# CLIAI/speaker-diarization-toolkit

Measured on AMD Instinct MI355X. Metric: segment-embeddings/sec, higher is better.
Workload: dtype bf16; 1 GPU; config #2: 1k synthetic 2-s segments/GPU -> fbank -> ECAPA-TDNN C=1024 -> L2 -> cosine argmax vs 100 profiles; segments_per_gpu=1000, embed_dim=192, weights=random-init seed 0 (20.77 M params), parallelism=segments sharded x1, profiles replicated

## Files before the change

### speaker-diarization-toolkit_amd/csrc/common.hpp

```cpp
#pragma once
#include <hip/hip_runtime.h>
#include <stdint.h>
#include <stdio.h>
#include <vector>

#include "../../include/sdk_hip.h"

typedef __bf16 bf16_t;
typedef __bf16 bf16x8 __attribute__((ext_vector_type(8)));
typedef __bf16 bf16x4 __attribute__((ext_vector_type(4)));
typedef __bf16 bf16x2 __attribute__((ext_vector_type(2)));
typedef float f32x4 __attribute__((ext_vector_type(4)));
typedef float f32x16 __attribute__((ext_vector_type(16)));
typedef uint32_t u32x4 __attribute__((ext_vector_type(4)));
typedef uint32_t u32x2 __attribute__((ext_vector_type(2)));

struct sdk_prof_rec {
  int family;
  hipEvent_t a, b;
  double flops, bytes;
};
struct sdk_ctx {
  int device;
  int num_cu;
  hipDeviceProp_t prop;
  bool prof_on = false;
  bool no_chain_fusion = false;
  bool no_chain_two_per_cu = false;
  bool no_chain_packed = false;
  bool no_asp_packed = false;
  bool no_asp_seg = false;
  bool no_h_kblocked = false;
  int precision = 0;
  int aff_fast = 1;
  void* dbg_ptr = nullptr;
  void* gemm_clk_ptr = nullptr;
  void* gemm_stamps_ptr = nullptr;
  int hp_gemm_variant = 0;
  int matvec_variant = 0;
  int aff_boundary_pen = 0;
  int chol_pivot_rtol_ppb = 1000;
  int chol_shift_ppb = 0;
  bool ahc_distances_only = false;
  bool snorm_scores_only = false;
  bool trials_no_hist = false;
  int aff_variant = 0;
  std::vector<const void*> lds_optin;
  std::vector<sdk_prof_rec> prof;
};

int sdk_lds_optin(sdk_ctx* ctx, const void* func, int bytes);

int asp_fused_launch(sdk_ctx* ctx, const uint16_t* ah, int64_t ldah, const uint16_t* w2, const uint16_t* w2p, const float* b2,
                     const uint16_t* h, int64_t ldh, int B, int T, int C, int A, float* pooled, void* stream, bool kblocked = false, bool f16 = false);

int se_gate_residual_impl(sdk_ctx* ctx, const uint16_t* z, int64_t ldz, const uint16_t* x, int64_t ldx, const float* w1t, const float* b1, const float* w2t,
                          const float* b2, uint16_t* out, int64_t ldo, int B, int T, int C, int Cse, const float* mean_in, void* ws, size_t ws_bytes,
                          void* stream, bool f16);
int asp_stats_impl(sdk_ctx* ctx, const uint16_t* h, int64_t ldh, int B, int T, int C, float* out_ctx, void* stream, bool f16);
int asp_pool_impl(sdk_ctx* ctx, const float* logits, int64_t ldl, const uint16_t* h, int64_t ldh, int B, int T, int C, float* pooled, void* stream, bool f16);

int asp_stats_masked_impl(sdk_ctx* ctx, const uint16_t* h, int64_t ldh, int B, int T, int C, int S, const float* w, const int32_t* valid, float* out_ctx,
                          void* stream, bool f16, int32_t* ok_out);
int asp_pool_masked_impl(sdk_ctx* ctx, const float* logits, int64_t ldl, const uint16_t* h, int64_t ldh, int B, int T, int C, int S, int s, const float* w,
                         const int32_t* valid, float* pooled, void* stream, bool f16);

int res2net_chain_launch(sdk_ctx* ctx, const uint16_t* U, int64_t ldu, uint16_t* R, int64_t ldr, const uint16_t* const* W,
                         const uint16_t* const* Wpk, const float* const* bias, const float* const* scale, const float* const* shift,
                         int nconv, int B, int T, int dil, void* stream, bool f16 = false);

int resnet_tstp_impl(sdk_ctx* ctx, const uint16_t* x, int B, int F, int T, int C, float* out, void* stream, bool f16);
int resnet_masked_tstp_impl(sdk_ctx* ctx, const uint16_t* x, int B, int F, int T, int C, int S, const float* w, const int32_t* valid, float* out,
                            void* stream, bool f16);
int resnet_zero_invalid_impl(sdk_ctx* ctx, float* emb, int n, int dim, const int32_t* valid, void* stream);

size_t ahc_workspace_bytes(const int32_t* offsets, int G);
int ahc_launch(sdk_ctx* ctx, const float* E, int ldE, int dim, const int32_t* offsets, int G, double* Z, int32_t* status, void* ws, void* stream);
int link_launch(sdk_ctx* ctx, const float* E, int ldE, int dim, const int32_t* group, const int32_t* offsets, int G, double stop, double* Z, int32_t* merges,
                int32_t* status, void* ws, void* stream);

struct ProfScope {
  sdk_ctx* c; hipStream_t s; size_t slot; bool on;
  ProfScope(sdk_ctx* ctx, void* stream, int family, double flops, double bytes) : c(ctx), s((hipStream_t)stream), slot(0), on(ctx && ctx->prof_on) {
    if (!on) return;
    sdk_prof_rec r{family, nullptr, nullptr, flops, bytes};
    (void)hipEventCreate(&r.a); (void)hipEventCreate(&r.b);
    (void)hipEventRecord(r.a, s);
    slot = c->prof.size();
    c->prof.push_back(r);
  }
  ~ProfScope() { if (on) (void)hipEventRecord(c->prof[slot].b, s); }
};

void sdk_set_error(const char* fmt, ...) __attribute__((format(printf, 1, 2)));

#define SDK_HIP_OK(expr)                                                              \
  do {                                                                                \
    hipError_t _e = (expr);                                                           \
    if (_e != hipSuccess) {                                                           \
      sdk_set_error("%s failed: %s (%s:%d)", #expr, hipGetErrorString(_e), __FILE__, __LINE__); \
      return 1;                                                                       \
    }                                                                                 \
  } while (0)

#define SDK_REQUIRE(cond, ...)            \
  do {                                    \
    if (!(cond)) {                        \
      sdk_set_error(__VA_ARGS__);         \
      return 2;                           \
    }                                     \
  } while (0)

#define SDK_LAUNCH_CHECK()                                                         \
  do {                                                                             \
    hipError_t _e = hipGetLastError();                                             \
    if (_e != hipSuccess) {                                                        \
      sdk_set_error("kernel launch failed: %s (%s:%d)", hipGetErrorString(_e), __FILE__, __LINE__); \
      return 1;                                                                    \
    }                                                                              \
  } while (0)

static inline int ceil_div(int a, int b) { return (a + b - 1) / b; }

__device__ __forceinline__ float bf16_to_f32(bf16_t v) { return (float)v; }
__device__ __forceinline__ bf16_t f32_to_bf16(float v) { return (bf16_t)v; }

__device__ __forceinline__ float bf16_bits_to_f32(uint32_t lo16) { return __uint_as_float(lo16 << 16); }

__device__ __forceinline__ void unpack8(const u32x4& v, float* f) {
#pragma unroll
  for (int i = 0; i < 4; ++i) {
    f[2 * i] = __uint_as_float(v[i] << 16);
    f[2 * i + 1] = __uint_as_float(v[i] & 0xffff0000u);
  }
}
__device__ __forceinline__ uint32_t pack2(float a, float b) {
  bf16x2 t;
  t[0] = (bf16_t)a;
  t[1] = (bf16_t)b;
  return __builtin_bit_cast(uint32_t, t);
}
typedef _Float16 f16x8_t __attribute__((ext_vector_type(8)));
typedef _Float16 f16x2_t __attribute__((ext_vector_type(2)));
__device__ __forceinline__ float sat_f16(float a) {
  const float c = fminf(fmaxf(a, -65504.f), 65504.f);
  return a != a ? a : c;
}
template <bool F16>
__device__ __forceinline__ uint32_t pack2t(float a, float b) {
  if constexpr (F16) {
    f16x2_t t;
    t[0] = (_Float16)sat_f16(a);
    t[1] = (_Float16)sat_f16(b);
    return __builtin_bit_cast(uint32_t, t);
  } else {
    return pack2(a, b);
  }
}
template <bool F16>
__device__ __forceinline__ void unpack8t(const u32x4& v, float* f) {
  if constexpr (F16) {
#pragma unroll
    for (int i = 0; i < 4; ++i) {
      const uint32_t w = v[i];
      const f16x2_t t = __builtin_bit_cast(f16x2_t, w);
      f[2 * i] = (float)t[0];
      f[2 * i + 1] = (float)t[1];
    }
  } else {
    unpack8(v, f);
  }
}

__device__ __forceinline__ u32x4 pack8(const float* f) {
  u32x4 v;
#pragma unroll
  for (int i = 0; i < 4; ++i) v[i] = pack2(f[2 * i], f[2 * i + 1]);
  return v;
}
template <bool F16>
__device__ __forceinline__ u32x4 pack8t(const float* f) {
  u32x4 v;
#pragma unroll
  for (int i = 0; i < 4; ++i) v[i] = pack2t<F16>(f[2 * i], f[2 * i + 1]);
  return v;
// ... 46 lines not shown
```

### speaker-diarization-toolkit_amd/csrc/conv_gemm.hip

```cpp
#include <stdlib.h>

#include <type_traits>

#include "common.hpp"
#ifndef SDK_GEMM_CHAIN2
#define SDK_GEMM_CHAIN2 2
#endif

namespace {

__device__ __forceinline__ float tanh_bf16(float x) { return 1.0f - __fdividef(2.0f, __expf(2.0f * x) + 1.0f); }

constexpr int BM = 128, BN = 128, BK = 64, NT = 256;
constexpr int LDS_AB = (BM + BN) * BK * 2;
constexpr int CT_STRIDE = (BN + 8) * 2;
constexpr int LDS_CT = BM * CT_STRIDE;
constexpr int LDS_BYTES = LDS_CT > LDS_AB ? LDS_CT : LDS_AB;

struct Params {
  const bf16_t* A; int64_t lda;
  const bf16_t* W;
  bf16_t* C; int64_t ldc;
  float* C32; int64_t ldc32;
  const float* bias; const float* scale; const float* shift;
// ... 37 lines not shown
    m = m < p.M ? m : p.M - 1;
    if (p.taps > 1) {
      const int b = m / p.T;
      segbase[i] = b * p.T;
      tloc[i] = m - b * p.T;
    } else {
      segbase[i] = m;
      tloc[i] = 0;
    }
  }
  const int cpt = p.tap_pack >> 3;
  const int cin_w = p.tap_pack ? BK : p.Cin;
  const int Ktot = p.tap_pack ? ((p.taps * p.tap_pack + BK - 1) / BK) * BK : p.taps * p.Cin;
  const bf16_t* wrow[4];
#pragma unroll
  for (int i = 0; i < 4; ++i) wrow[i] = p.W + (int64_t)(n0 + r0 + 32 * i) * Ktot + ch * 8;

  uint32_t lds_w[4];
#pragma unroll
  for (int i = 0; i < 4; ++i) {
    const int row = r0 + 32 * i;
    lds_w[i] = row * 128 + ((ch ^ (row & 7)) << 4);
  }

  const int ksteps_per_tap = cin_w / BK;
  const int nk = p.tap_pack ? Ktot / BK : p.taps * ksteps_per_tap;
  const int half = p.taps >> 1;

  u32x4 ra[4], rb[4], ra2[4];
  auto gload = [&](int s) {
    const int j = s / ksteps_per_tap;
    const int kc = (s - j * ksteps_per_tap) * BK;
    int off = (j - half) * p.dil, acol = kc + ch * 8;
    if (p.tap_pack) {
      const int g = s * 8 + ch;
      int tap = g / cpt;
      acol = (g - tap * cpt) * 8;
      if (tap >= p.taps) { tap = half; acol = 0; }
      off = (tap - half) * p.dil;
    }
#pragma unroll
    for (int i = 0; i < 4; ++i) {
      const int src = p.taps > 1 ? segbase[i] + reflect_idx(tloc[i] + off, p.T) : segbase[i];
      ra[i] = *reinterpret_cast<const u32x4*>(p.ablk ? p.A + (int64_t)(acol >> 6) * p.ablk + (int64_t)src * 64 + (acol & 63) : p.A + (int64_t)src * p.lda + acol);
      rb[i] = *reinterpret_cast<const u32x4*>(wrow[i] + j * cin_w + kc);
      if (p.A2) ra2[i] = *reinterpret_cast<const u32x4*>(p.A2 + (int64_t)src * p.lda2 + acol);
    }
  };

  f32x4 acc[4][4];
#pragma unroll
  for (int mi = 0; mi < 4; ++mi)
#pragma unroll
    for (int ni = 0; ni < 4; ++ni) acc[mi][ni] = f32x4{0.f, 0.f, 0.f, 0.f};

  const int fr = lane & 15, fq = lane >> 4;
  uint32_t a_off[4], b_off[4];
#pragma unroll
  for (int i = 0; i < 4; ++i) {
    a_off[i] = (wm * 64 + i * 16 + fr) * 128;
    b_off[i] = (wn * 64 + i * 16 + fr) * 128;
  }
  const int sw = lane & 7;

  gload(0);
  for (int s = 0; s < nk; ++s) {
#pragma unroll
    for (int i = 0; i < 4; ++i) {
      if (p.A2) {
        float fa[8], fb[8];
        unpack8t<F16>(ra[i], fa);
        unpack8t<F16>(ra2[i], fb);
#pragma unroll
        for (int e = 0; e < 8; ++e) fa[e] += fb[e];
        ra[i] = pack8t<F16>(fa);
      }
      *reinterpret_cast<u32x4*>(sA + lds_w[i]) = ra[i];
      *reinterpret_cast<u32x4*>(sB + lds_w[i]) = rb[i];
    }
    __syncthreads();
    if (s + 1 < nk) gload(s + 1);
#pragma unroll
    for (int ks = 0; ks < 2; ++ks) {
      const uint32_t coff = ((ks * 4 + fq) ^ sw) << 4;
      bf16x8 af[4], bfr[4];
#pragma unroll
      for (int i = 0; i < 4; ++i) {
        af[i] = *reinterpret_cast<const bf16x8*>(sA + a_off[i] + coff);
        bfr[i] = *reinterpret_cast<const bf16x8*>(sB + b_off[i] + coff);
      }
#pragma unroll
      for (int mi = 0; mi < 4; ++mi)
#pragma unroll
        for (int ni = 0; ni < 4; ++ni)
          acc[mi][ni] = mfma_16x16x32<F16>(af[mi], bfr[ni], acc[mi][ni]);
    }
    __syncthreads();
  }

  float cb[4], cs[4], ct[4];
#pragma unroll
  for (int ni = 0; ni < 4; ++ni) {
    const int col = n0 + wn * 64 + ni * 16 + fr;
    cb[ni] = p.bias ? p.bias[col] : 0.f;
    cs[ni] = p.scale ? p.scale[col] : 1.f;
    ct[ni] = p.shift ? p.shift[col] : 0.f;
  }
  const bool relu = p.flags & SDK_GEMM_RELU, tnh = p.flags & SDK_GEMM_TANH;
#pragma unroll
  for (int mi = 0; mi < 4; ++mi) {
#pragma unroll
    for (int r = 0; r < 4; ++r) {
      const int row = wm * 64 + mi * 16 + fq * 4 + r;
      const int m = m0 + row;
      const float* ub = nullptr;
      if (p.ubias) {
        const int mm = m < p.M ? m : p.M - 1;
        ub = p.ubias + (int64_t)(mm / p.T) * p.ldub;
      }
#pragma unroll
      for (int ni = 0; ni < 4; ++ni) {
        const int lc = wn * 64 + ni * 16 + fr;
        float v = acc[mi][ni][r] + cb[ni];
        if (ub) v += ub[n0 + lc];
        if (relu) v = fmaxf(v, 0.f);
        v = v * cs[ni] + ct[ni];
        if (tnh) v = tanh_bf16(v);
        if (p.C32 && m < p.M) p.C32[(int64_t)m * p.ldc32 + n0 + lc] = v;
        *reinterpret_cast<uint16_t*>(smem + row * CT_STRIDE + lc * 2) = (uint16_t)pack2t<F16>(v, 0.f);
      }
    }
  }
  __syncthreads();
  if (p.C || p.S) {
#pragma unroll
    for (int i = 0; i < 8; ++i) {
      const int id = tid + NT * i;
      const int row = id >> 4, cc = id & 15;
      const int m = m0 + row;
      if (m < p.M) {
        const u32x4 v = *reinterpret_cast<const u32x4*>(smem + row * CT_STRIDE + cc * 16);
        if (p.C) *reinterpret_cast<u32x4*>(p.C + (int64_t)m * p.ldc + n0 + cc * 8) = v;
        if (p.S) {
          const u32x4 x = *reinterpret_cast<const u32x4*>(p.X2 + (int64_t)m * p.ldx2 + n0 + cc * 8);
          float fv[8], fx[8];
          unpack8t<F16>(v, fv);
          unpack8t<F16>(x, fx);
#pragma unroll
          for (int e = 0; e < 8; ++e) fv[e] += fx[e];
          *reinterpret_cast<u32x4*>(p.S + (int64_t)m * p.lds + n0 + cc * 8) = pack8t<F16>(fv);
        }
      }
    }
  }
}

}

namespace {

constexpr int BM2 = 256, BN2 = 256, NT2 = 512;
constexpr int STAGE2 = (BM2 + BN2) * BK * 2;
constexpr int LDS2 = 2 * STAGE2;
constexpr int LDS2_PAR = LDS2 + 3 * BN2 * 4;
constexpr int LDS2_TOTAL = LDS2_PAR + 8 * 2 * BN2 * 4;
static_assert(BM2 * BN2 * 2 <= LDS2, "the bf16 image of a finished tile must fit in the two pipeline stages");

typedef const void __attribute__((address_space(1)))* gptr_t;
typedef void __attribute__((address_space(3)))* lptr_t;

template <bool TAPS, bool CKB = false, bool F16 = false>
__global__ __launch_bounds__(NT2, 2) void conv_gemm256_kernel(Params p) {
  extern __shared__ __attribute__((aligned(16))) char smem[];
  const int tid = threadIdx.x, lane = tid & 63, wid = tid >> 6;
  const unsigned long long clk_c0 = p.clk ? __builtin_amdgcn_s_memtime() : 0, clk_r0 = p.clk ? __builtin_amdgcn_s_memrealtime() : 0;
  const int wm = wid >> 2, wn = wid & 3;

  const int nbn = p.N / BN2;
  const int nbm = (p.M + BM2 - 1) / BM2;
  const int ntiles = nbn * nbm;
  const int cpt = p.tap_pack >> 3;
  const int cin_w = p.tap_pack ? BK : p.Cin;
  const int Ktot = p.tap_pack ? ((p.taps * p.tap_pack + BK - 1) / BK) * BK : p.taps * p.Cin;
  const int ksteps_per_tap = cin_w / BK;
  const int nk = p.tap_pack ? Ktot / BK : p.taps * ksteps_per_tap;
  const int half = p.taps >> 1;

  const int G = gridDim.x;
  const bool unit_order = !(p.tune & 64) && G == 256 && (nbn & 3) == 0 && nbm >= 64;
  const int xcd = blockIdx.x & 7, slot = blockIdx.x >> 3;
  const int nch = nbn >> 2, mg_full = nbm >> 3;
  const int full_units = mg_full * nch, R = full_units >> 3, rem_units = full_units - 8 * R;
  const int gm_tail = nbm & 7, tail_tiles = gm_tail * nbn;
  const int mt0 = unit_order && (8 * R) % nch == 0 ? ((8 * R) / nch) * 8 : 0;
  const int n_half_m = 2 * (nbm - mt0);
  const int half_cap = 32 / nbn;
  const bool half_tail = unit_order && !(p.tune & 512) && (8 * R) % nch == 0 && R > 0 && mt0 < nbm && n_half_m <= 8 * half_cap;
  const int nrounds = unit_order ? (half_tail ? R : R + (rem_units + (tail_tiles + 31) / 32 + 7) / 8) : (ntiles + G - 1) / G;
  auto tile_coords = [&](int i, int& tm0, int& tn0) -> bool {
    if (unit_order) {
      int u;
      if (i < R) {
        u = xcd * R + i;
      } else {
        const int q = (i - R) * 8 + xcd;
        if (q >= rem_units) {
          const int pj = (q - rem_units) * 32 + slot;
          if (pj >= tail_tiles) return false;
          tm0 = (mg_full * 8 + pj % gm_tail) * BM2;
          tn0 = (pj / gm_tail) * BN2;
          return true;
        }
        u = 8 * R + q;
      }
      const int mg = u / nch, ch = u - mg * nch;
      tm0 = (mg * 8 + (slot & 7)) * BM2;
      tn0 = (ch * 4 + (slot >> 3)) * BN2;
      return true;
    }
    const int vt = blockIdx.x + G * i;
    if (vt >= ntiles) return false;
    const int tile = xcd_remap(vt, ntiles);
    constexpr int GM = 8;
    const int per_group = GM * nbn;
    const int grp = tile / per_group, in_grp = tile - grp * per_group;
    const int gm = min(nbm - grp * GM, GM);
    tm0 = (grp * GM + in_grp % gm) * BM2;
    tn0 = (in_grp / gm) * BN2;
    return true;
  };

  const int rin = lane >> 3, pos = lane & 7;
  const int gch = (pos ^ rin) * 8;
  const int wu = __builtin_amdgcn_readfirstlane(wid);
  const bool a_nt = !TAPS && nbn <= 4;
  uint32_t aoff[4];
  int aseg0 = 0, atl0 = 0;
  uint32_t woff;
  auto setup_dma = [&](int tm0, int tn0, auto ap_c) {
    constexpr int AP = decltype(ap_c)::value;
    const int row = 8 * AP * wu + rin;
    if constexpr (TAPS) {
      const int mm = min(tm0 + row, p.M - 1);
      aseg0 = (mm / p.T) * p.T;
      atl0 = mm - aseg0;
    } else {
#pragma unroll
      for (int i = 0; i < AP; ++i) aoff[i] = ((uint32_t)min(tm0 + row + 8 * i, p.M - 1) * (uint32_t)p.lda + (uint32_t)gch) * 2u;
    }
    woff = ((uint32_t)(tn0 + 32 * wu + rin) * (uint32_t)Ktot + (uint32_t)gch) * 2u;
  };
  auto issue = [&](int t, int stage, auto ap_c) {
    constexpr int AP = decltype(ap_c)::value;
    const int j = t / ksteps_per_tap;
    const int kc = (t - j * ksteps_per_tap) * BK;
    char* sA = smem + stage * STAGE2 + (8 * AP * wu) * 128;
    char* sB = smem + stage * STAGE2 + BM2 * BK * 2 + (32 * wu) * 128;
    const char* abase = reinterpret_cast<const char*>(p.A + kc);
    if constexpr (TAPS) {
      int off = (j - half) * p.dil;
      uint32_t acol = (uint32_t)gch;
      if (p.tap_pack) {
        const int g = t * 8 + (gch >> 3);
        int tap = g / cpt;
        acol = (uint32_t)(g - tap * cpt) * 8u;
        if (tap >= p.taps) { tap = half; acol = 0; }
        off = (tap - half) * p.dil;
      }
#pragma unroll
      for (int i = 0; i < AP; ++i) {
        int tl = atl0 + 8 * i, sb = aseg0;
        if (tl >= p.T) { tl -= p.T; sb += p.T; }
        const uint32_t src = (uint32_t)min(sb + reflect_idx(tl + off, p.T), p.M - 1);
        __builtin_amdgcn_global_load_lds((gptr_t)(abase + (size_t)((src * (uint32_t)p.lda + acol) * 2u)), (lptr_t)(sA + i * 1024), 16, 0, 0);
      }
    } else if (a_nt) {
#pragma unroll
      for (int i = 0; i < AP; ++i)
        __builtin_amdgcn_global_load_lds((gptr_t)(abase + (size_t)aoff[i]), (lptr_t)(sA + i * 1024), 16, 0, 2);
    } else {
#pragma unroll
      for (int i = 0; i < AP; ++i)
        __builtin_amdgcn_global_load_lds((gptr_t)(abase + (size_t)aoff[i]), (lptr_t)(sA + i * 1024), 16, 0, 0);
    }
    const char* wbase = reinterpret_cast<const char*>(p.W + (j * cin_w + kc));
#pragma unroll
    for (int i = 0; i < 4; ++i)
      __builtin_amdgcn_global_load_lds((gptr_t)(wbase + (size_t)i * 16 * Ktot + (size_t)woff), (lptr_t)(sB + i * 1024), 16, 0, 0);
  };
  constexpr std::integral_constant<int, 4> kWhole{};
  constexpr std::integral_constant<int, 2> kHalf{};

  const int fr = lane & 15, fq = lane >> 4, sw = lane & 7;
  const uint32_t a_base = (wm * 128 + fr) * 128;
  const uint32_t b_base = BM2 * BK * 2 + (wn * 64 + fr) * 128;
  const uint32_t c0 = ((0 * 4 + fq) ^ sw) << 4, c1 = ((1 * 4 + fq) ^ sw) << 4;
  const bool dma_early = wu < 4;
  const bool relu = p.flags & SDK_GEMM_RELU;
  const bool stats = p.stats_part != nullptr;
  float* par = reinterpret_cast<float*>(smem + LDS2);

  int nst = 0;
  auto stamp = [&]() {
    if (p.stamps && blockIdx.x == 0 && tid == 0 && nst < 4096) p.stamps[nst++] = __builtin_amdgcn_s_memrealtime();
  };
  auto ldB = [&](const char* st, bf16x8* dst, uint32_t coff) {
// ... 418 lines not shown
      bf16_t* dst = CKB ? p.C + (int64_t)((n0 >> 6) + (cc >> 3)) * p.cblk + (int64_t)(m0 + r0) * 64 + (cc & 7) * 8
                        : p.C + (int64_t)(m0 + r0) * p.ldc + n0 + cc * 8;
      const int64_t ldc = CKB ? 64 : p.ldc;
      const int rows_left = p.M - m0 - r0;
#pragma unroll
      for (int i = 0; i < 8; ++i) {
        if (16 * i < rows_left) {
          const u32x4 v = *reinterpret_cast<const u32x4*>(src + i * 16 * (BN2 * 2));
          __builtin_nontemporal_store(v, reinterpret_cast<u32x4*>(dst + (int64_t)(16 * i) * ldc));
        }
      }
    }
    if (stats) tile_stats((m0 / BM2) * BM2, m0 & 128, 128, n0);
    stamp();
    }
  }
  if (p.clk && tid == 0 && blockIdx.x < 4096) {
    p.clk[blockIdx.x * 2] = __builtin_amdgcn_s_memtime() - clk_c0;
    p.clk[blockIdx.x * 2 + 1] = __builtin_amdgcn_s_memrealtime() - clk_r0;
  }
}

__global__ __launch_bounds__(256) void colstats_finish_kernel(const float* __restrict__ part, int M, int N, int T, int mode,
                                                             float* __restrict__ out) {
  const int b = blockIdx.x, n = blockIdx.y * 256 + threadIdx.x;
  if (n >= N) return;
  const int64_t nbm = (M + BM2 - 1) / BM2;
  const int r_lo = b * T, r_hi = (b + 1) * T - 1;
  float s = 0.f, q = 0.f;
  for (int t = r_lo / BM2; t <= r_hi / BM2; ++t) {
    const int slot = b - (t * BM2) / T;
    const float* ps = part + ((int64_t)(t * 2) * 3 + slot) * N + n;
    s += ps[0];
    s += ps[3 * (int64_t)N];
    if (mode == 2) {
      const float* pq = ps + nbm * 6 * N;
      q += pq[0];
      q += pq[3 * (int64_t)N];
    }
  }
  const float invT = 1.0f / (float)T;
  const float mean = s * invT;
  if (mode == 1) {
    out[(int64_t)b * N + n] = mean;
  } else {
    out[(int64_t)b * 2 * N + n] = mean;
    out[(int64_t)b * 2 * N + N + n] = sqrtf(var_floor(q * invT - mean * mean));
  }
}

int g_gemm_variant = -1;

}

extern "C" size_t sdk_conv_gemm_stats_bytes(int M, int N, int mode) {
  if (M <= 0 || N <= 0 || mode < 1 || mode > 2) return 0;
  return (size_t)((M + BM2 - 1) / BM2) * 6 * (size_t)N * sizeof(float) * (size_t)mode;
}

extern "C" int sdk_conv_gemm_stats_fusable(int M, int N, int T) {
  return ((g_gemm_variant < 0 ? 2 : g_gemm_variant) & 15) != 1 && N % BN2 == 0 && M >= BM2 && T >= 128;
}

extern "C" int sdk_colstats_finish(sdk_ctx* ctx, const float* stats_part, int M, int N, int T, int mode, float* out, void* stream) {
  SDK_REQUIRE(ctx && stats_part && out, "sdk_colstats_finish: null argument");
  SDK_REQUIRE(M > 0 && T > 0 && M % T == 0 && (mode == 1 || mode == 2), "sdk_colstats_finish: bad shape");
  hipLaunchKernelGGL(colstats_finish_kernel, dim3(M / T, ceil_div(N, 256)), dim3(256), 0, (hipStream_t)stream, stats_part, M, N, T, mode, out);
  SDK_LAUNCH_CHECK();
  return 0;
}

extern "C" int sdk_set_gemm_variant(int v) {
  g_gemm_variant = v;
  return 0;
}

extern "C" int sdk_conv_gemm(sdk_ctx* ctx, const sdk_conv_gemm_args* a, void* stream) {
  SDK_REQUIRE(ctx && a, "sdk_conv_gemm: null ctx/args");
  SDK_REQUIRE(a->A && a->W, "sdk_conv_gemm: A and W are required");
  SDK_REQUIRE(a->M > 0 && a->N > 0 && a->N % BN == 0, "sdk_conv_gemm: N=%d must be a positive multiple of %d", a->N, BN);
  const int pack = a->tap_pack;
  if (pack) {
    SDK_REQUIRE(pack > 0 && pack % 8 == 0 && a->taps > 1 && !a->A2 && a->Cin == pack, "sdk_conv_gemm: tap_pack=%d needs taps > 1, a multiple of 8 channels per tap, Cin == tap_pack and no A2", pack);
  } else
  SDK_REQUIRE(a->Cin > 0 && a->Cin % BK == 0, "sdk_conv_gemm: Cin=%d must be a multiple of %d", a->Cin, BK);
  SDK_REQUIRE(a->taps >= 1 && (a->taps & 1), "sdk_conv_gemm: taps=%d must be odd", a->taps);
  SDK_REQUIRE(a->T > 0 && a->M % a->T == 0, "sdk_conv_gemm: M=%d must be a multiple of T=%d", a->M, a->T);
  SDK_REQUIRE((int64_t)a->N * a->taps * a->Cin < (1ll << 31), "sdk_conv_gemm: weight matrix of %d x %d elements exceeds 2^31", a->N, a->taps * a->Cin);
  SDK_REQUIRE(a->taps == 1 || (a->taps / 2) * a->dil < a->T, "sdk_conv_gemm: segment of T=%d frames shorter than the conv halo %d", a->T, (a->taps / 2) * a->dil);
  const bool a_kb = (a->flags & SDK_GEMM_A_KBLOCKED) != 0, c_kb = (a->flags & SDK_GEMM_C_KBLOCKED) != 0, f16 = (a->flags & SDK_GEMM_F16) != 0;
  if (a_kb) SDK_REQUIRE(a->taps == 1 && !pack && !a->A2, "sdk_conv_gemm: a K-blocked A operand needs taps == 1, no tap packing and no A2");
  else
  SDK_REQUIRE(a->lda % 8 == 0 && a->lda >= a->Cin, "sdk_conv_gemm: lda=%lld must be >= Cin and a multiple of 8", (long long)a->lda);
  SDK_REQUIRE(((uintptr_t)a->A % 16) == 0 && ((uintptr_t)a->W % 16) == 0, "sdk_conv_gemm: A/W must be 16-byte aligned");
  SDK_REQUIRE(a->C || a->C32 || a->S, "sdk_conv_gemm: no output requested");
  if (a->C && !c_kb) SDK_REQUIRE(a->ldc % 8 == 0 && a->ldc >= a->N && ((uintptr_t)a->C % 16) == 0, "sdk_conv_gemm: bad C/ldc");
  if (c_kb) SDK_REQUIRE(a->C && ((uintptr_t)a->C % 16) == 0, "sdk_conv_gemm: a K-blocked output needs C (16-byte aligned)");
  if (a->S) SDK_REQUIRE(a->X2 && a->lds % 8 == 0 && a->ldx2 % 8 == 0 && ((uintptr_t)a->S % 16) == 0 && ((uintptr_t)a->X2 % 16) == 0, "sdk_conv_gemm: S needs X2 and 16-byte aligned rows");
  if (a->C32) SDK_REQUIRE(a->ldc32 >= a->N, "sdk_conv_gemm: bad ldc32");
  if (a->ubias) SDK_REQUIRE(a->ldub >= a->N, "sdk_conv_gemm: bad ldub");

  if (g_gemm_variant < 0) {
    const char* e = getenv("SDK_GEMM_VARIANT");
    g_gemm_variant = e ? atoi(e) : 2;
  }
  if (sdk_lds_optin(ctx, (const void*)conv_gemm256_kernel<false>, LDS2_TOTAL)) return 1;
  if (sdk_lds_optin(ctx, (const void*)conv_gemm256_kernel<true>, LDS2_TOTAL)) return 1;
  if (sdk_lds_optin(ctx, (const void*)conv_gemm256_kernel<false, true>, LDS2_TOTAL)) return 1;
  if (sdk_lds_optin(ctx, (const void*)conv_gemm256_kernel<false, false, true>, LDS2_TOTAL)) return 1;
  if (sdk_lds_optin(ctx, (const void*)conv_gemm256_kernel<true, false, true>, LDS2_TOTAL)) return 1;
  if (sdk_lds_optin(ctx, (const void*)conv_gemm256_kernel<false, true, true>, LDS2_TOTAL)) return 1;
  Params p;
  p.A = (const bf16_t*)a->A; p.lda = a->lda; p.W = (const bf16_t*)a->W;
  p.C = (bf16_t*)a->C; p.ldc = a->ldc; p.C32 = a->C32; p.ldc32 = a->ldc32;
  p.bias = a->bias; p.scale = a->scale; p.shift = a->shift; p.ubias = a->ubias; p.ldub = a->ldub;
  p.X2 = (const bf16_t*)a->X2; p.ldx2 = a->ldx2; p.S = (bf16_t*)a->S; p.lds = a->lds;
  p.M = a->M; p.N = a->N; p.Cin = a->Cin; p.taps = a->taps; p.dil = a->dil; p.T = a->T; p.flags = a->flags;
  p.tune = g_gemm_variant / 16;
  p.stats_part = nullptr; p.stats_mode = 0;
  p.A2 = (const bf16_t*)a->A2; p.lda2 = a->lda2;
  p.tap_pack = pack;
  p.ablk = a_kb ? (int64_t)a->M * 64 : 0;
  p.cblk = c_kb ? (int64_t)a->M * 64 : 0;
  p.clk = (unsigned long long*)ctx->gemm_clk_ptr;
  p.stamps = (unsigned long long*)ctx->gemm_stamps_ptr;
  if (a->A2) SDK_REQUIRE(a->lda2 % 8 == 0 && a->lda2 >= a->Cin && ((uintptr_t)a->A2 % 16) == 0, "sdk_conv_gemm: bad A2/lda2");

  const double kk = pack ? (double)(((a->taps * pack + BK - 1) / BK) * BK) : (double)a->taps * a->Cin;
  const bool use256 = !a_kb && ((g_gemm_variant & 15) != 1 || c_kb) && a->N % BN2 == 0 && a->M >= BM2 && !a->A2 && a->C && !a->C32 && !a->S &&
                      !a->ubias && !(a->flags & SDK_GEMM_TANH) && (a->taps == 1 || a->T >= 64) &&
                      (uint64_t)a->M * (uint64_t)a->lda * 2u < (1ull << 32);
  ProfScope ps(ctx, stream, use256 ? SDK_K_CONV_GEMM256 : SDK_K_CONV_GEMM, 2.0 * a->M * a->N * kk,
               2.0 * a->M * a->Cin + 2.0 * a->N * kk + (a->C ? 2.0 : 0.0) * a->M * a->N + (a->C32 ? 4.0 : 0.0) * a->M * a->N +
                   (a->S ? 4.0 : 0.0) * a->M * a->N);
  if (c_kb) SDK_REQUIRE(use256 && a->taps == 1, "sdk_conv_gemm: a K-blocked output needs the plain-layer shape of the 256^2 kernel (taps == 1, N %% 256 == 0, M >= 256, bf16 output only)");
  if (a->stats_mode) {
    SDK_REQUIRE(a->stats_mode == 1 || a->stats_mode == 2, "sdk_conv_gemm: stats_mode=%d", a->stats_mode);
    SDK_REQUIRE(use256 && a->T >= 128 && a->stats_part && a->C, "sdk_conv_gemm: fused column statistics need the 256^2 kernel (N %% 256 == 0, M >= 256), T >= 128 and a bf16 output");
    p.stats_part = a->stats_part; p.stats_mode = a->stats_mode;
  }
  if (use256) {
    const int ntiles = (a->N / BN2) * ceil_div(a->M, BM2);
    const int cus = ctx->num_cu > 0 ? (ctx->num_cu / 8) * 8 : 256;
    const int grid = (p.tune & 8) ? ntiles : (ntiles < cus ? ntiles : cus);
    if (f16) {
      void (*kern)(Params) = conv_gemm256_kernel<false, false, true>;
      if (c_kb) kern = conv_gemm256_kernel<false, true, true>;
      else if (p.taps > 1) kern = conv_gemm256_kernel<true, false, true>;
      hipLaunchKernelGGL(kern, dim3(grid), dim3(NT2), LDS2_TOTAL, (hipStream_t)stream, p);
    } else if (c_kb)
      hipLaunchKernelGGL((conv_gemm256_kernel<false, true>), dim3(grid), dim3(NT2), LDS2_TOTAL, (hipStream_t)stream, p);
    else
      hipLaunchKernelGGL(p.taps > 1 ? conv_gemm256_kernel<true> : conv_gemm256_kernel<false>, dim3(grid), dim3(NT2), LDS2_TOTAL, (hipStream_t)stream, p);
  } else {
    hipLaunchKernelGGL(f16 ? conv_gemm_kernel<true> : conv_gemm_kernel<false>, dim3((a->N / BN) * ceil_div(a->M, BM)), dim3(NT), LDS_BYTES, (hipStream_t)stream, p);
  }
  SDK_LAUNCH_CHECK();
  return 0;
}
```

### speaker-diarization-toolkit_amd/csrc/sdk_api.hip

```cpp
#include <stdarg.h>
#include <string.h>

#include "common.hpp"
#include "ecapa_layout.h"
#include "hp.hpp"

static thread_local char g_err[512] = "";

void sdk_set_error(const char* fmt, ...) {
  va_list ap;
  va_start(ap, fmt);
  vsnprintf(g_err, sizeof(g_err), fmt, ap);
  va_end(ap);
}

extern "C" const char* sdk_last_error(void) { return g_err; }
extern "C" int sdk_abi_version(void) { return SDK_ABI_VERSION; }

extern "C" int sdk_init(int device, sdk_ctx** out) {
  SDK_REQUIRE(out, "sdk_init: out is null");
  *out = nullptr;
  int n = 0;
  hipError_t e = hipGetDeviceCount(&n);
  if (e != hipSuccess || n <= 0) {
    sdk_set_error("sdk_init: no HIP device available (%s); this library has no CPU fallback",
                  e != hipSuccess ? hipGetErrorString(e) : "device count is 0");
    return 1;
  }
  SDK_REQUIRE(device >= 0 && device < n, "sdk_init: device %d out of range (0..%d)", device, n - 1);
  sdk_ctx* c = new sdk_ctx();
  c->device = device;
  if (hipGetDeviceProperties(&c->prop, device) != hipSuccess) {
    delete c;
    sdk_set_error("sdk_init: hipGetDeviceProperties failed");
    return 1;
  }
  if (strncmp(c->prop.gcnArchName, "gfx950", 6) != 0) {
    sdk_set_error("sdk_init: device %d is %s; libsdk_hip.so carries gfx950 (MI355X) code objects only", device,
                  c->prop.gcnArchName);
    delete c;
    return 1;
  }
  c->num_cu = c->prop.multiProcessorCount;
  SDK_HIP_OK(hipSetDevice(device));
  *out = c;
  return 0;
}

int sdk_lds_optin(sdk_ctx* ctx, const void* func, int bytes) {
  for (const void* f : ctx->lds_optin)
    if (f == func) return 0;
  SDK_HIP_OK(hipSetDevice(ctx->device));
  SDK_HIP_OK(hipFuncSetAttribute(func, hipFuncAttributeMaxDynamicSharedMemorySize, bytes));
  ctx->lds_optin.push_back(func);
  return 0;
}

extern "C" int sdk_device_malloc(sdk_ctx* ctx, size_t bytes, void** out) {
  SDK_REQUIRE(ctx && out, "sdk_device_malloc: null argument");
  *out = nullptr;
  SDK_HIP_OK(hipSetDevice(ctx->device));
  SDK_HIP_OK(hipMalloc(out, bytes ? bytes : 1));
  return 0;
}
extern "C" int sdk_device_free(sdk_ctx* ctx, void* p) {
  SDK_REQUIRE(ctx, "sdk_device_free: null context");
  if (p) SDK_HIP_OK(hipFree(p));
  return 0;
}
extern "C" int sdk_memcpy(sdk_ctx* ctx, void* dst, const void* src, size_t bytes, int kind, void* stream) {
  SDK_REQUIRE(ctx && (bytes == 0 || (dst && src)), "sdk_memcpy: null argument");
  SDK_REQUIRE(kind >= 1 && kind <= 3, "sdk_memcpy: kind=%d (1 = host to device, 2 = device to host, 3 = device to device)", kind);
  if (!bytes) return 0;
  const hipMemcpyKind k = kind == 1 ? hipMemcpyHostToDevice : kind == 2 ? hipMemcpyDeviceToHost : hipMemcpyDeviceToDevice;
  SDK_HIP_OK(hipMemcpyAsync(dst, src, bytes, k, (hipStream_t)stream));
  SDK_HIP_OK(hipStreamSynchronize((hipStream_t)stream));
  return 0;
}
extern "C" int sdk_stream_synchronize(sdk_ctx* ctx, void* stream) {
  SDK_REQUIRE(ctx, "sdk_stream_synchronize: null context");
  SDK_HIP_OK(hipStreamSynchronize((hipStream_t)stream));
  return 0;
}

extern "C" int sdk_shutdown(sdk_ctx* ctx) {
  delete ctx;
  return 0;
}

extern "C" int sdk_get_device_info(sdk_ctx* ctx, sdk_device_info* out) {
  SDK_REQUIRE(ctx && out, "sdk_get_device_info: null argument");
  memset(out, 0, sizeof(*out));
  out->device = ctx->device;
  out->compute_units = ctx->prop.multiProcessorCount;
  out->clock_khz = ctx->prop.clockRate;
  out->wavefront_size = ctx->prop.warpSize;
  out->hbm_bytes = ctx->prop.totalGlobalMem;
  strncpy(out->name, ctx->prop.name, sizeof(out->name) - 1);
  strncpy(out->arch, ctx->prop.gcnArchName, sizeof(out->arch) - 1);
  return 0;
}

extern "C" int sdk_set_option(sdk_ctx* ctx, const char* name, int value) {
  SDK_REQUIRE(ctx && name, "sdk_set_option: null argument");
  if (strcmp(name, "res2net_chain_fusion") == 0) { ctx->no_chain_fusion = value == 0; return 0; }
  if (strcmp(name, "res2net_packed_weights") == 0) { ctx->no_chain_packed = value == 0; return 0; }
  if (strcmp(name, "res2net_two_per_cu") == 0) { ctx->no_chain_two_per_cu = value == 0; return 0; }
  if (strcmp(name, "asp_packed_weights") == 0) { ctx->no_asp_packed = value == 0; return 0; }
  if (strcmp(name, "asp_per_segment") == 0) { ctx->no_asp_seg = value == 0; return 0; }
  if (strcmp(name, "h_kblocked") == 0) { ctx->no_h_kblocked = value == 0; return 0; }
  if (strcmp(name, "precision") == 0) {
    SDK_REQUIRE(value >= 0 && value <= 2, "sdk_set_option: precision must be 0 (bf16 operands), 1 (fp16 hi+lo planes) or 2 (one fp16 plane), got %d", value);
    ctx->precision = value;
    return 0;
  }
  if (strcmp(name, "gemm_variant") == 0) return sdk_set_gemm_variant(value);
  if (strcmp(name, "affinity_fast_path") == 0) { ctx->aff_fast = value; return 0; }
  if (strcmp(name, "affinity_variant") == 0) { ctx->aff_variant = value; return 0; }
  if (strcmp(name, "affinity_boundary_penalty") == 0) { ctx->aff_boundary_pen = value < 0 ? 0 : value; return 0; }
  if (strcmp(name, "matvec_variant") == 0) { ctx->matvec_variant = value; return 0; }
  if (strcmp(name, "hp_gemm_variant") == 0) { ctx->hp_gemm_variant = value; return 0; }
  if (strcmp(name, "affinity_whole_groups") == 0) return 0;
  if (strcmp(name, "chol_pivot_rtol_ppb") == 0) { ctx->chol_pivot_rtol_ppb = value < 0 ? 0 : value; return 0; }
  if (strcmp(name, "chol_shift_ppb") == 0) { ctx->chol_shift_ppb = value < 0 ? 0 : value; return 0; }
  if (strcmp(name, "ahc_distances_only") == 0) { ctx->ahc_distances_only = value != 0; return 0; }
  if (strcmp(name, "snorm_scores_only") == 0) { ctx->snorm_scores_only = value != 0; return 0; }
  if (strcmp(name, "trials_no_hist") == 0) { ctx->trials_no_hist = value != 0; return 0; }
  sdk_set_error("sdk_set_option: unknown option '%s'", name);
  return 2;
}

extern "C" int sdk_debug_set_ptr(sdk_ctx* ctx, const char* name, void* p) {
  SDK_REQUIRE(ctx && name, "sdk_debug_set_ptr: null argument");
  if (strcmp(name, "stamps") == 0) { ctx->dbg_ptr = p; return 0; }
  if (strcmp(name, "gemm_clock") == 0) { ctx->gemm_clk_ptr = p; return 0; }
  if (strcmp(name, "gemm_stamps") == 0) { ctx->gemm_stamps_ptr = p; return 0; }
  sdk_set_error("sdk_debug_set_ptr: unknown name '%s'", name);
  return 2;
}

extern "C" int sdk_profile_begin(sdk_ctx* ctx) {
  SDK_REQUIRE(ctx, "sdk_profile_begin: null ctx");
  for (auto& r : ctx->prof) { (void)hipEventDestroy(r.a); (void)hipEventDestroy(r.b); }
  ctx->prof.clear();
  ctx->prof_on = true;
  return 0;
}

extern "C" int sdk_profile_end(sdk_ctx* ctx, sdk_profile_report* out) {
  SDK_REQUIRE(ctx && out, "sdk_profile_end: null argument");
  ctx->prof_on = false;
  memset(out, 0, sizeof(*out));
  SDK_HIP_OK(hipDeviceSynchronize());
  for (auto& r : ctx->prof) {
    float ms = 0.f;
    SDK_HIP_OK(hipEventElapsedTime(&ms, r.a, r.b));
    if (r.family >= 0 && r.family < SDK_K_COUNT) {
      out->launches[r.family] += 1;
      out->ms[r.family] += ms;
      out->flops[r.family] += r.flops;
      out->bytes[r.family] += r.bytes;
    }
    (void)hipEventDestroy(r.a);
    (void)hipEventDestroy(r.b);
  }
  ctx->prof.clear();
  return 0;
}

namespace {

inline size_t a256(size_t v) { return (v + 255) & ~(size_t)255; }

struct FwdWs {
  uint16_t *X0, *U, *R, *Z, *Sa, *Sb, *CAT, *H, *AH;
  float *ctx, *ubias, *logits, *pooled, *se, *stats, *mean;
};

size_t fwd_layout(const sdk_ecapa_desc* d, int B, int T, char* base, FwdWs* w, bool full_logits = false) {
  const size_t M = (size_t)B * T, C = d->channels, Cm = d->mfa_channels, S = d->sub_channels, A = d->attn_channels;
  size_t off = 0;
  auto take = [&](size_t bytes) { char* p = base ? base + off : nullptr; off += a256(bytes); return p; };
  char* x0 = take(M * C * 2);
  char* u = take(M * C * 2);
  char* r = take(M * C * 2);
  char* z = take(M * C * 2);
  char* sa = take(M * S * 2);
  char* sb = take(M * S * 2);
  char* cat = take(M * Cm * 2);
  char* h = take(M * Cm * 2);
  char* ah = take(M * A * 2);
  char* cx = take((size_t)B * 2 * Cm * 4);
  char* ub = take((size_t)B * A * 4);
  const bool fused_asp = !full_logits && A == 128 && T <= sdk_asp_fused_max_frames();
  char* lg = take(fused_asp ? 256 : M * Cm * 4);
  char* po = take((size_t)B * 2 * Cm * 4);
  char* se = take(sdk_se_workspace_bytes(B, (int)C, d->se_channels));
  char* stp = take(sdk_conv_gemm_stats_bytes((int)M, (int)Cm, 2));
  char* mn = take((size_t)B * C * 4);
  if (w) { w->se = (float*)se; w->stats = (float*)stp; w->mean = (float*)mn; }
  if (w) {
    w->X0 = (uint16_t*)x0; w->U = (uint16_t*)u; w->R = (uint16_t*)r; w->Z = (uint16_t*)z;
    w->Sa = (uint16_t*)sa; w->Sb = (uint16_t*)sb; w->CAT = (uint16_t*)cat; w->H = (uint16_t*)h; w->AH = (uint16_t*)ah;
    w->ctx = (float*)cx; w->ubias = (float*)ub; w->logits = (float*)lg; w->pooled = (float*)po;
  }
  return off;
}

struct FwdWsHp {
  uint16_t *X0, *U, *R, *Z, *Sa, *Sb, *CAT, *H, *AH;
  float *ctx, *ubias, *logits, *pooled, *mean, *hid, *gate;
};

size_t fwd_layout_hp(const sdk_ecapa_desc* d, int B, int T, char* base, FwdWsHp* w) {
  const size_t M = (size_t)B * T, C = d->channels, Cm = d->mfa_channels, S = d->sub_channels, A = d->attn_channels;
  size_t off = 0;
  auto take = [&](size_t bytes) { char* p = base ? base + off : nullptr; off += a256(bytes); return p; };
  char* x0 = take(M * C * 4);
  char* u = take(M * C * 4);
  char* r = take(M * C * 4);
  char* z = take(M * C * 4);
  char* sa = take(M * S * 4);
  char* sb = take(M * S * 4);
  char* cat = take(M * Cm * 4);
  char* h = take(M * Cm * 4);
  char* ah = take(M * A * 4);
  char* cx = take((size_t)B * 2 * Cm * 4);
  char* ub = take((size_t)B * A * 4);
  char* lg = take(M * Cm * 4);
  char* po = take((size_t)B * 2 * Cm * 4);
  char* mn = take((size_t)B * C * 4);
  char* hd = take((size_t)B * d->se_channels * 4);
  char* gt = take((size_t)B * C * 4);
  if (w) {
    w->X0 = (uint16_t*)x0; w->U = (uint16_t*)u; w->R = (uint16_t*)r; w->Z = (uint16_t*)z; w->Sa = (uint16_t*)sa; w->Sb = (uint16_t*)sb;
    w->CAT = (uint16_t*)cat; w->H = (uint16_t*)h; w->AH = (uint16_t*)ah; w->ctx = (float*)cx; w->ubias = (float*)ub; w->logits = (float*)lg;
    w->pooled = (float*)po; w->mean = (float*)mn; w->hid = (float*)hd; w->gate = (float*)gt;
  }
  return off;
}

int check_desc(const sdk_ecapa_desc* d) {
  SDK_REQUIRE(d, "ecapa desc is null");
  SDK_REQUIRE(d->n_blocks >= 1 && d->n_blocks <= 4, "ecapa desc: n_blocks=%d", d->n_blocks);
  SDK_REQUIRE(d->channels % 128 == 0 && d->mfa_channels == d->n_blocks * d->channels, "ecapa desc: channels=%d mfa=%d", d->channels, d->mfa_channels);
  SDK_REQUIRE(d->scale >= 2 && d->sub_channels * d->scale == d->channels && d->sub_channels % 128 == 0, "ecapa desc: res2net scale=%d sub=%d", d->scale, d->sub_channels);
  SDK_REQUIRE(d->attn_channels % 128 == 0 && d->n_mels_padded % (d->precision == 1 ? 32 : 64) == 0, "ecapa desc: attn=%d mels=%d", d->attn_channels, d->n_mels_padded);
  SDK_REQUIRE((d->kernel0 & 1) == 1, "ecapa desc: kernel0=%d must be odd", d->kernel0);
  SDK_REQUIRE(d->precision >= 0 && d->precision <= 2, "ecapa desc: precision=%d", d->precision);
  return 0;
}

int ecapa_forward_hp(sdk_ctx* ctx, const void* wblob, const sdk_ecapa_desc* d, const uint16_t* feats, int ldf, int B, int T, void* ws,
                     float* emb, void* stream) {
  FwdWsHp w;
  fwd_layout_hp(d, B, T, (char*)ws, &w);
  const char* wb = (const char*)wblob;
  auto P16 = [&](int slot) -> const uint16_t* { return d->off[slot] < 0 ? nullptr : (const uint16_t*)(wb + d->off[slot]); };
  auto P32 = [&](int slot) -> const float* { return d->off[slot] < 0 ? nullptr : (const float*)(wb + d->off[slot]); };
  const int M = B * T, C = d->channels, Cm = d->mfa_channels, S = d->sub_channels, A = d->attn_channels;
  const int flo = ldf >> 1;
  SDK_REQUIRE(ldf % 16 == 0 && flo >= d->n_mels_padded, "sdk_ecapa_forward: precise mode takes feature planes, ldf=%d must be >= 2 x %d", ldf, d->n_mels_padded);

// ... 614 lines not shown
```

Baseline: 121,400 segment-embeddings/sec.

## Add persistent double-buffered skinny GEMM kernel for N=128 convolutions

```diff
diff --git a/speaker-diarization-toolkit_amd/csrc/common.hpp b/speaker-diarization-toolkit_amd/csrc/common.hpp
--- a/speaker-diarization-toolkit_amd/csrc/common.hpp
+++ b/speaker-diarization-toolkit_amd/csrc/common.hpp
@@ -31,6 +31,7 @@
   bool no_asp_packed = false;
   bool no_asp_seg = false;
   bool no_h_kblocked = false;
+  bool no_skinny_gemm = false;
   int precision = 0;
   int aff_fast = 1;
   void* dbg_ptr = nullptr;
diff --git a/speaker-diarization-toolkit_amd/csrc/conv_gemm.hip b/speaker-diarization-toolkit_amd/csrc/conv_gemm.hip
--- a/speaker-diarization-toolkit_amd/csrc/conv_gemm.hip
+++ b/speaker-diarization-toolkit_amd/csrc/conv_gemm.hip
@@ -213,6 +213,183 @@
         }
       }
     }
+  }
+}
+
+constexpr int SK_LDS = 2 * LDS_AB;
+static_assert(BM * BN * 2 <= LDS_AB, "the 2-byte image of a finished tile must fit in one pipeline stage");
+
+template <bool F16>
+__global__ __launch_bounds__(NT, 2) void conv_gemm_skinny_kernel(Params p) {
+  extern __shared__ __attribute__((aligned(16))) char smem[];
+  const int tid = threadIdx.x;
+  const int lane = tid & 63;
+  const int wid = tid >> 6;
+  const int wm = wid >> 1, wn = wid & 1;
+
+  const int ntiles = (p.M + BM - 1) / BM;
+  const int G = gridDim.x;
+  const int nk = p.Cin / BK;
+  const int total = ((ntiles - (int)blockIdx.x + G - 1) / G) * nk;
+
+  const int ch = tid & 7;
+  const int r0 = tid >> 3;
+  const uint32_t lds_w0 = r0 * 128 + ((ch ^ (r0 & 7)) << 4);
+  const int64_t arow = p.ablk ? 64 : p.lda;
+  const int64_t astep_live = p.ablk ? p.ablk : BK;
+
+  const bf16_t* pa[4];
+  int64_t astep = 0;
+  int a_vt = blockIdx.x, a_k = 0;
+  auto a_tile = [&]() __attribute__((always_inline)) {
+    const bool live = a_vt < ntiles;
+    const int m0 = live ? xcd_remap(a_vt, ntiles) * BM : 0;
+    astep = live ? astep_live : 0;
+#pragma unroll
+    for (int i = 0; i < 4; ++i) {
+      int m = m0 + r0 + 32 * i;
+      m = m < p.M ? m : p.M - 1;
+      pa[i] = p.A + (live ? (int64_t)m * arow : 0) + ch * 8;
+    }
+  };
+  auto a_issue = [&](u32x4* dst) __attribute__((always_inline)) {
+#pragma unroll
+    for (int i = 0; i < 4; ++i) {
+      dst[i] = *reinterpret_cast<const u32x4*>(pa[i]);
+      pa[i] += astep;
+    }
+    if (++a_k == nk) { a_k = 0; a_vt += G; a_tile(); }
+  };
+  a_tile();
+  const bf16_t* const w0 = p.W + (int64_t)r0 * p.Cin + ch * 8;
+  const int64_t wrow32 = (int64_t)32 * p.Cin;
+  int w_k = 0;
+  auto w_issue = [&](u32x4* dst) __attribute__((always_inline)) {
+#pragma unroll
+    for (int i = 0; i < 4; ++i) dst[i] = *reinterpret_cast<const u32x4*>(w0 + i * wrow32 + w_k * BK);
+    w_k = w_k + 1 == nk ? 0 : w_k + 1;
+  };
+  auto lds_fill = [&](char* stage, const u32x4* a, const u32x4* b) __attribute__((always_inline)) {
+#pragma unroll
+    for (int i = 0; i < 4; ++i) *reinterpret_cast<u32x4*>(stage + lds_w0 + i * 4096) = a[i];
+    __builtin_amdgcn_sched_barrier(0);
+#pragma unroll
+    for (int i = 0; i < 4; ++i) *reinterpret_cast<u32x4*>(stage + BM * BK * 2 + lds_w0 + i * 4096) = b[i];
+    __builtin_amdgcn_sched_barrier(0);
+  };
+
+  f32x4 acc[4][4];
+#pragma unroll
+  for (int mi = 0; mi < 4; ++mi)
+#pragma unroll
+    for (int ni = 0; ni < 4; ++ni) acc[mi][ni] = f32x4{0.f, 0.f, 0.f, 0.f};
+
+  const int fr = lane & 15, fq = lane >> 4;
+  uint32_t a_off[4], b_off[4];
+#pragma unroll
+  for (int i = 0; i < 4; ++i) {
+    a_off[i] = (wm * 64 + i * 16 + fr) * 128;
+    b_off[i] = BM * BK * 2 + (wn * 64 + i * 16 + fr) * 128;
+  }
+  const int sw = lane & 7;
+
+  const bool relu = p.flags & SDK_GEMM_RELU, tnh = p.flags & SDK_GEMM_TANH;
+
+  auto epilogue = [&](int m0, char* img) __attribute__((always_inline)) {
+    float cb[4], cs[4], ct[4];
+#pragma unroll
+    for (int ni = 0; ni < 4; ++ni) {
+      const int col = wn * 64 + ni * 16 + fr;
+      cb[ni] = p.bias ? p.bias[col] : 0.f;
+      cs[ni] = p.scale ? p.scale[col] : 1.f;
+      ct[ni] = p.shift ? p.shift[col] : 0.f;
+    }
+    const bool has_ub = p.ubias != nullptr;
+#pragma unroll
+    for (int mi = 0; mi < 4; ++mi) {
+      float ubv[4][4];
+#pragma unroll
+      for (int r = 0; r < 4; ++r) {
+        const int m = m0 + wm * 64 + mi * 16 + fq * 4 + r;
+        const int mm = m < p.M ? m : p.M - 1;
+        const float* ub = has_ub ? p.ubias + (int64_t)(mm / p.T) * p.ldub : nullptr;
+#pragma unroll
+        for (int ni = 0; ni < 4; ++ni) ubv[r][ni] = has_ub ? ub[wn * 64 + ni * 16 + fr] : 0.f;
+      }
+#pragma unroll
+      for (int r = 0; r < 4; ++r) {
+        const int row = wm * 64 + mi * 16 + fq * 4 + r;
+#pragma unroll
+        for (int ni = 0; ni < 4; ++ni) {
+          const int lc = wn * 64 + ni * 16 + fr;
+          float v = acc[mi][ni][r] + cb[ni];
+          if (has_ub) v += ubv[r][ni];
+          if (relu) v = fmaxf(v, 0.f);
+          v = v * cs[ni] + ct[ni];
+          if (tnh) v = tanh_bf16(v);
+          *reinterpret_cast<uint16_t*>(img + row * 256 + (((lc >> 3) ^ (fq << 1)) << 4) + (lc & 7) * 2) = (uint16_t)pack2t<F16>(v, 0.f);
+          acc[mi][ni][r] = 0.f;
+        }
+      }
+    }
+    lds_barrier();
+#pragma unroll
+    for (int i = 0; i < 8; ++i) {
+      const int id = tid + NT * i;
+      const int row = id >> 4, cc = id & 15;
+      const int m = m0 + row;
+      if (m < p.M) {
+        const u32x4 v = *reinterpret_cast<const u32x4*>(img + row * 256 + ((cc ^ (((row >> 2) & 3) << 1)) << 4));
+        *reinterpret_cast<u32x4*>(p.C + (int64_t)m * p.ldc + cc * 8) = v;
+      }
+    }
+    lds_barrier();
+  };
+
+  u32x4 ra[2][4], rb[4];
+  int c_vt = blockIdx.x, c_k = 0;
+  auto step = [&](auto par_c) __attribute__((always_inline)) {
+    constexpr int P = decltype(par_c)::value;
+    char* st = smem + P * LDS_AB;
+    lds_fill(smem + (P ^ 1) * LDS_AB, ra[P ^ 1], rb);
+    w_issue(rb);
+    a_issue(ra[P ^ 1]);
+    __builtin_amdgcn_sched_barrier(0);
+#pragma unroll
+    for (int ks = 0; ks < 2; ++ks) {
+      const uint32_t coff = ((ks * 4 + fq) ^ sw) << 4;
+      bf16x8 af[4], bfr[4];
+#pragma unroll
+      for (int i = 0; i < 4; ++i) {
+        af[i] = *reinterpret_cast<const bf16x8*>(st + a_off[i] + coff);
+        bfr[i] = *reinterpret_cast<const bf16x8*>(st + b_off[i] + coff);
+      }
+#pragma unroll
+      for (int mi = 0; mi < 4; ++mi)
+#pragma unroll
+        for (int ni = 0; ni < 4; ++ni)
+          acc[mi][ni] = mfma_16x16x32<F16>(af[mi], bfr[ni], acc[mi][ni]);
+    }
+    lds_barrier();
+    if (++c_k == nk && c_vt < ntiles) {
+      epilogue(xcd_remap(c_vt, ntiles) * BM, st);
+      c_k = 0;
+      c_vt += G;
+    }
+  };
+  constexpr std::integral_constant<int, 0> kEven{};
+  constexpr std::integral_constant<int, 1> kOdd{};
+
+  a_issue(ra[0]);
+  w_issue(rb);
+  a_issue(ra[1]);
+  lds_fill(smem, ra[0], rb);
+  w_issue(rb);
+  a_issue(ra[0]);
+  lds_barrier();
+  for (int g = 0; g < total; g += 2) {
+    step(kEven);
+    step(kOdd);
   }
 }
 
@@ -937,6 +1114,11 @@
       hipLaunchKernelGGL((conv_gemm256_kernel<false, true>), dim3(grid), dim3(NT2), LDS2_TOTAL, (hipStream_t)stream, p);
     else
       hipLaunchKernelGGL(p.taps > 1 ? conv_gemm256_kernel<true> : conv_gemm256_kernel<false>, dim3(grid), dim3(NT2), LDS2_TOTAL, (hipStream_t)stream, p);
+  } else if (!ctx->no_skinny_gemm && a->N == BN && a->taps == 1 && !pack && !a->A2 && !a->X2 && !a->S && !a->C32 && a->C && !a->stats_mode) {
+    const int ntiles = ceil_div(a->M, BM);
+    const int slots = 2 * (ctx->num_cu >= 8 ? (ctx->num_cu / 8) * 8 : 256);
+    hipLaunchKernelGGL(f16 ? conv_gemm_skinny_kernel<true> : conv_gemm_skinny_kernel<false>, dim3(ntiles < slots ? ntiles : slots), dim3(NT), SK_LDS,
+                       (hipStream_t)stream, p);
   } else {
     hipLaunchKernelGGL(f16 ? conv_gemm_kernel<true> : conv_gemm_kernel<false>, dim3((a->N / BN) * ceil_div(a->M, BM)), dim3(NT), LDS_BYTES, (hipStream_t)stream, p);
   }
diff --git a/speaker-diarization-toolkit_amd/csrc/sdk_api.hip b/speaker-diarization-toolkit_amd/csrc/sdk_api.hip
--- a/speaker-diarization-toolkit_amd/csrc/sdk_api.hip
+++ b/speaker-diarization-toolkit_amd/csrc/sdk_api.hip
@@ -109,6 +109,7 @@
   if (strcmp(name, "asp_packed_weights") == 0) { ctx->no_asp_packed = value == 0; return 0; }
   if (strcmp(name, "asp_per_segment") == 0) { ctx->no_asp_seg = value == 0; return 0; }
   if (strcmp(name, "h_kblocked") == 0) { ctx->no_h_kblocked = value == 0; return 0; }
+  if (strcmp(name, "skinny_gemm") == 0) { ctx->no_skinny_gemm = value == 0; return 0; }
   if (strcmp(name, "precision") == 0) {
     SDK_REQUIRE(value >= 0 && value <= 2, "sdk_set_option: precision must be 0 (bf16 operands), 1 (fp16 hi+lo planes) or 2 (one fp16 plane), got %d", value);
     ctx->precision = value;
```

Measured after the change: 121,000 segment-embeddings/sec. No clear change (-0.4%).
